# jewettaij/visfd

Hardware: AMD Instinct MI355X
Metric: Mvoxels/s (Gauss+DoG+TV pipeline) on 1024^3 float32; % HBM roofline (higher is better)
Workload: dtype f32

## Files before the change

visfd_amd/build.py:

```python
import concurrent.futures
import os
import subprocess
import sys
import time

HERE = os.path.dirname(os.path.abspath(__file__))
ROOT = os.path.dirname(HERE)
CSRC = os.path.join(HERE, "csrc")
OBJDIR = os.path.join(ROOT, "build", "visfd_hip")
LIB = os.path.join(HERE, "libvisfd_hip.so")

SOURCES = ["host_math.cpp", "blob_post.cpp", "connect.cpp", "watershed_host.cpp", "context.hip", "api.hip", "blob_job.hip", "gauss.hip", "blob.hip", "select.hip", "tv.hip", "resample.hip", "slab.hip", "morph.hip", "extrema.hip", "filter3d.hip", "draw.hip", "watershed.hip", "median.hip", "intensity.hip", "distance.hip"]
TV_VARIANT = [("tv_tiled.hip", "tv_tiled", ["-fno-slp-vectorize"]), ("tv_box.hip", "tv_box", ["-fno-slp-vectorize"]),
              ("tv_list.hip", "tv_list", ["-fno-slp-vectorize"]),
              ("ridge.hip", "ridge", [])]
VARIANTS = TV_VARIANT + [("gauss_fused.hip", "gauss_fused_h%d" % h, ["-DVH_FUSED_H=%d" % h, "-fno-slp-vectorize"])
                         for h in range(1, 9)]
HEADERS = ["common.hpp", "tv_common.hpp", "eigen3.hpp", "union_find.hpp", "tile.hpp", "watershed_host.hpp", "intensity.hpp", os.path.join("..", "..", "include", "visfd_hip.h")]

HIPCC = os.environ.get("HIPCC", "/opt/rocm/bin/hipcc")
FLAGS = ["--offload-arch=gfx950", "-O3", "-std=c++17", "-fPIC", "-ffp-contract=off", "-fno-fast-math",
         "-Wall", "-Wno-unused-function"]


def _mtime(p):
    return os.path.getmtime(p) if os.path.exists(p) else 0.0


def _compile(src, obj, extra=()):
    t0 = time.time()
    cmd = [HIPCC] + FLAGS + list(extra) + ["-x", "hip", "-c", os.path.join(CSRC, src), "-o", obj]
    r = subprocess.run(cmd, capture_output=True, text=True)
    return src, r.returncode, r.stdout + r.stderr, time.time() - t0


def build(force=False, jobs=4, verbose=True):
    os.makedirs(OBJDIR, exist_ok=True)
    newest_header = max(_mtime(os.path.join(CSRC, h)) for h in HEADERS)
    todo, objs = [], []
    units = [(s, os.path.splitext(s)[0], []) for s in SOURCES] + VARIANTS
    flagfile = os.path.join(OBJDIR, "flags.txt")
    flagsig = repr((FLAGS, VARIANTS))
    if not os.path.exists(flagfile) or open(flagfile).read() != flagsig:
        force = True
    for s, stem, extra in units:
        obj = os.path.join(OBJDIR, stem + ".o")
        objs.append(obj)
        if force or _mtime(obj) < max(_mtime(os.path.join(CSRC, s)), newest_header):
            todo.append((s, obj, extra))
    if todo:
        with concurrent.futures.ThreadPoolExecutor(max_workers=jobs) as ex:
            for (src, rc, out, dt), (_, obj, _e) in zip(ex.map(lambda a: _compile(*a), todo), todo):
                if verbose:
                    print("[visfd_amd.build] %-22s %5.1fs %s" % (os.path.basename(obj), dt, "ok" if rc == 0 else "FAILED"))
                if rc != 0:
                    sys.stderr.write(out)
                    raise RuntimeError("hipcc failed on " + src)
                elif out.strip() and verbose:
                    sys.stderr.write(out)
    with open(flagfile, "w") as f:
        f.write(flagsig)
    if todo or not os.path.exists(LIB) or _mtime(LIB) < max(_mtime(o) for o in objs):
        cmd = [HIPCC, "--offload-arch=gfx950", "-shared", "-fPIC", "-o", LIB] + objs
        r = subprocess.run(cmd, capture_output=True, text=True)
        if r.returncode != 0:
            sys.stderr.write(r.stdout + r.stderr)
            raise RuntimeError("link failed")
        if verbose:
            print("[visfd_amd.build] linked", LIB)
    build_cli(verbose)
    return LIB


CLI_SRC = os.path.join(HERE, "cli", "filter_mrc.cpp")
CLI_BIN = os.path.join(HERE, "cli", "filter_mrc")


def build_cli(verbose=True):
    deps = [CLI_SRC, os.path.join(HERE, "cli", "mrc.hpp"), os.path.join(HERE, "cli", "settings.hpp"),
            os.path.join(ROOT, "include", "visfd_hip.hpp"), os.path.join(ROOT, "include", "visfd_hip.h"), LIB]
    if os.path.exists(CLI_BIN) and _mtime(CLI_BIN) >= max(_mtime(d) for d in deps):
        return CLI_BIN
    cmd = ["g++", "-std=c++11", "-O2", "-Wall", "-o", CLI_BIN, CLI_SRC, "-L" + HERE, "-lvisfd_hip",
           "-Wl,-rpath,$ORIGIN/..", "-Wl,-rpath,/opt/rocm/lib"]
    r = subprocess.run(cmd, capture_output=True, text=True)
    if r.returncode != 0:
        sys.stderr.write(r.stdout + r.stderr)
        raise RuntimeError("building filter_mrc failed")
    if verbose:
        print("[visfd_amd.build] built", CLI_BIN)
    return CLI_BIN


if __name__ == "__main__":
    j = 4
    if "-j" in sys.argv:
        j = int(sys.argv[sys.argv.index("-j") + 1])
    build(force="--force" in sys.argv, jobs=j)
```

visfd_amd/csrc/api.hip:

```cpp
#include <algorithm>
#include <cmath>
#include <vector>

#include "common.hpp"

namespace vh {

int gauss_dev(visfd_hip_ctx* ctx, const float* src, float* dst, const float* mask, i64 nx, i64 ny, i64 nz,
              const float sigma[3], const int hw[3], bool normalize, const GaussOpts& o) {
  VH_REQUIRE(ctx && src && dst && sigma && hw, "null argument");
  std::vector<float> t[3];
  for (int d = 0; d < 3; d++) {
    VH_REQUIRE(sigma[d] >= 0.0f, "sigma must be non-negative");
    VH_REQUIRE(hw[d] >= 0 && hw[d] <= MAX_HALFWIDTH, "filter halfwidth must be in [0, 64]");
    t[d].resize(2 * hw[d] + 1);
    host_gauss_taps(sigma[d], hw[d], t[d].data());
  }
  return dev_separable3d(ctx, src, dst, mask, nx, ny, nz, t[0].data(), hw[0], t[1].data(), hw[1], t[2].data(), hw[2],
                         normalize, o);
}

static int dog_dev(visfd_hip_ctx* ctx, const float* src, float* dst, const float* mask, i64 nx, i64 ny, i64 nz,
                   const float sa[3], const float sb[3], const int hw[3], float scale, float* A, float* B) {
  VH_TRY(gauss_dev(ctx, src, dst, mask, nx, ny, nz, sa, hw, true, {A}));
  return gauss_dev(ctx, src, dst, mask, nx, ny, nz, sb, hw, true, {B, dst, scale});
}

LogPlan plan_log(const float sigma[3], float delta, float ratio) {
  LogPlan p;
  for (int d = 0; d < 3; d++) {
    p.sa[d] = (float)(sigma[d] * (1.0 - 0.5 * delta));
    p.sb[d] = (float)(sigma[d] * (1.0 + 0.5 * delta));
    p.hw[d] = (int)std::floor(ratio * std::fmax(p.sa[d], p.sb[d]));
  }
  p.scale = (float)(1.0 / (delta * delta));
  return p;
}

int log_dev(visfd_hip_ctx* ctx, const float* src, float* dst, const float* mask, i64 nx, i64 ny, i64 nz,
            const float sigma[3], float delta, float ratio, float* A, float* B) {
  const LogPlan p = plan_log(sigma, delta, ratio);
  for (int d = 0; d < 3; d++)
    VH_REQUIRE(p.hw[d] >= 0 && p.hw[d] <= MAX_HALFWIDTH, "LoG filter halfwidth must be in [0, 64]");
  float a = 0, b = 0;
  VH_TRY(dog_dev(ctx, src, dst, mask, nx, ny, nz, p.sa, p.sb, p.hw, p.scale, &a, &b));
  if (A) *A = a * p.scale;
  if (B) *B = b * p.scale;
  return VISFD_HIP_OK;
}

namespace {

void halfwidths_from_ratio(const float sigma[3], float ratio, int hw[3]) {
  for (int d = 0; d < 3; d++) {
    hw[d] = (int)std::floor(sigma[d] * ratio);
    if (hw[d] < 1) hw[d] = 1;
  }
}

int gauss_iso_dev(visfd_hip_ctx* ctx, const float* src, float* dst, const float* mask, i64 nx, i64 ny, i64 nz, float sigma,
                  float ratio, bool normalize, const char* what, float** out = nullptr) {
  const int hwv = (int)std::floor(sigma * ratio);
  VH_REQUIRE(hwv >= 0 && hwv <= MAX_HALFWIDTH, std::string(what) + " must be in [0, 64]");
  if (!dst) VH_TRY(ws(ctx, WS_D, (size_t)(nx * ny * nz), &dst));
  if (out) *out = dst;
  const float sg[3] = {sigma, sigma, sigma};
  const int hw[3] = {hwv, hwv, hwv};
  return gauss_dev(ctx, src, dst, mask, nx, ny, nz, sg, hw, normalize);
}

int calc_hessian_dev(visfd_hip_ctx* ctx, const float* src, float* grad, float* hess, const float* mask,
                     i64 nx, i64 ny, i64 nz, float sigma, float ratio) {
  VH_REQUIRE(ctx && src, "null argument");
  VH_TRY(check_dims(nx, ny, nz));
  float* S = nullptr;
  VH_TRY(gauss_iso_dev(ctx, src, nullptr, mask, nx, ny, nz, sigma, ratio, true, "filter halfwidth", &S));
  return dev_hessian(ctx, S, mask, nx, ny, nz, sigma, grad, hess);
}

GaussOpts field_opts(const visfd_hip_ctx* ctx, float* A_out) {
  GaussOpts o;
  o.A_out = A_out;
  o.fma = ctx->opt.gauss_fma != 0;
  return o;
}

bool overlaps(const float* a, const float* b, i64 n) { return a && b && a < b + n && b < a + n; }

int morph_check(visfd_hip_ctx* ctx, const float* src, float* dst, const float* mask, i64 nx, i64 ny, i64 nz, int op,
                int max_op) {
  VH_REQUIRE(ctx && src && dst, "null argument");
  VH_REQUIRE(op >= 0 && op <= max_op, "unknown morphology op");
  VH_TRY(check_dims(nx, ny, nz));
  VH_REQUIRE(!overlaps(src, dst, nx * ny * nz), "morphology cannot run in place (dst overlaps src)");
  VH_REQUIRE(!overlaps(mask, dst, nx * ny * nz), "morphology: dst overlaps mask");
  VH_HIP(hipSetDevice(ctx->device));
  return VISFD_HIP_OK;
}

int median_check(visfd_hip_ctx* ctx, const float* src, float* dst, const float* mask, i64 nx, i64 ny, i64 nz) {
  VH_REQUIRE(ctx && src && dst, "null argument");
  VH_TRY(check_dims(nx, ny, nz));
  VH_REQUIRE(!overlaps(src, dst, nx * ny * nz), "the median filter cannot run in place (dst overlaps src)");
  VH_REQUIRE(!overlaps(mask, dst, nx * ny * nz), "median: dst overlaps mask");
  VH_HIP(hipSetDevice(ctx->device));
  return VISFD_HIP_OK;
// ... 674 lines not shown
```

visfd_amd/csrc/common.hpp:

```cpp
#pragma once

#include <hip/hip_runtime.h>

#include <cstdint>
#include <cstdio>
#include <cstring>
#include <string>
#include <vector>

#include "../../include/visfd_hip.h"

namespace vh {

typedef int64_t i64;

void set_error(const std::string& msg);
int fail(int code, const std::string& msg);

#define VH_HIP(expr)                                                                         \
  do {                                                                                       \
    hipError_t _e = (expr);                                                                  \
    if (_e != hipSuccess)                                                                    \
      return vh::fail(_e == hipErrorOutOfMemory ? VISFD_HIP_ENOMEM : VISFD_HIP_EDEVICE,      \
                      std::string(#expr) + ": " + hipGetErrorString(_e));                    \
  } while (0)

#define VH_TRY(expr)           \
  do {                         \
    int _rc = (expr);          \
    if (_rc != VISFD_HIP_OK) return _rc; \
  } while (0)

#define VH_REQUIRE(cond, msg) \
  do {                        \
    if (!(cond)) return vh::fail(VISFD_HIP_EINVAL, msg); \
  } while (0)

enum Slot {
  WS_A = 0, WS_B, WS_C, WS_D,
  WS_DEN_A, WS_DEN_B,
  WS_NORM,
  WS_LOG0, WS_LOG1, WS_LOG2,
  WS_CAND, WS_COUNTER,
  WS_SCANCNT,
  WS_HIST,
  WS_TVTAB,
  WS_TVAUX,
  WS_TVSCRATCH,
  WS_TVLIST,
  WS_H2D_0, WS_H2D_1, WS_H2D_2, WS_H2D_3, WS_H2D_4,
  WS_MORPH_TAB,
  WS_MORPH_SRC,
  WS_MORPH_TMP,
  WS_EXT_FLAGS,
  WS_EXT_PARENT,
  WS_EXT_COUNT,
  WS_EXT_COUNTERS,
  WS_EXT_LIST,
  WS_EXT_RANKS,
  WS_F3D_TAB,
  WS_DRAW_OWNER,
  WS_DRAW_TAB,
  WS_WSH_KIND,
  WS_WSH_LINK,
  WS_WSH_C,
  WS_WSH_STATE,
  WS_WSH_SEEDS,
  WS_WSH_FLAGS,
  WS_MEDIAN_TAB,
  WS_INTENSITY,
  WS_DIST_DSQ,
  WS_DIST_STACK,
  WS_DIST_POINTS,
  WS_NSLOTS
};

struct BlobJob;

}

struct visfd_hip_options {
  int gauss_3pass = 0;
  int gauss_cfg = 0;
  int gauss_wg_per_cu = 2;
  int tv_dense = 0;
  int tv_fma = 0;
  int gauss_fma = 0;
  int eig_f32 = 0;
  int tv_zrun = 0;
  int tv_no_replay = 0;
  int tv_exact_tiled = 0;
  int tv_no_fold = 0;
  int tv_poison = 0;
  int tv_reserve_wg = 0;
  int tv_max_wg = 0;
  int64_t blob_test_cap = 0;
  int morph_general = 0;
  int filter3d_general = 0;
  int median_general = 0;
  int distance_general = 0;
  int watershed_host = 0;
  int stats_blocks = 0;
  int draw_time = 0;
  int debug = 0;
};

struct visfd_hip_ctx {
  visfd_hip_options opt;
  float* tv_table_dev = nullptr;
  float tv_table_key[2] = {0.0f, 0.0f};
  int tv_table_h = -1;
  int device = 0;
  hipStream_t stream = nullptr;
  bool own_stream = false;
  void* slot_ptr[vh::WS_NSLOTS] = {};
  size_t slot_bytes[vh::WS_NSLOTS] = {};
  int num_cus = 256;
  hipStream_t aux_stream = nullptr;
  std::vector<int> morph_tab;
  int morph_last_path = -1;
  std::vector<float> f3d_raw;
  int64_t f3d_key[5] = {};
  int64_t f3d_n = 0;
  int64_t f3d_ncols = 0;
  float f3d_den = 0.0f;
  int f3d_last_path = -1;
  std::vector<int> median_tab;
  int median_last_path = -1;
  int distance_last_path = -1;
  float draw_ms[3] = {-1.0f, -1.0f, -1.0f};
  int64_t wsh_stats[4] = {-1, -1, -1, -1};
  std::vector<vh::BlobJob*> blob_jobs;
};

namespace vh {

int blob_jobs_drain(visfd_hip_ctx* ctx, const BlobJob* except = nullptr);
void blob_jobs_abort(visfd_hip_ctx* ctx);

int ws_get(visfd_hip_ctx* ctx, Slot s, size_t bytes, void** out);
template <typename T>
inline int ws(visfd_hip_ctx* ctx, Slot s, size_t count, T** out) {
  void* p = nullptr;
  int rc = ws_get(ctx, s, count * sizeof(T), &p);
  *out = static_cast<T*>(p);
  return rc;
}

inline int check_dims(i64 nx, i64 ny, i64 nz) {
  if (nx <= 0 || ny <= 0 || nz <= 0) return fail(VISFD_HIP_EINVAL, "image dimensions must be positive");
  return VISFD_HIP_OK;
}
inline bool overlap_bytes(const void* a, size_t na, const void* b, size_t nb) {
  const char* p = static_cast<const char*>(a);
  const char* q = static_cast<const char*>(b);
  return p && q && p < q + nb && q < p + na;
}
inline int check_dims32(i64 nx, i64 ny, i64 nz) {
  if (nx >= (1LL << 31) || ny >= (1LL << 31) || nz >= (1LL << 31)) return fail(VISFD_HIP_EINVAL, "dimension too large");
  return VISFD_HIP_OK;
}

constexpr int MAX_HALFWIDTH = 64;
struct Taps {
  float t[2 * MAX_HALFWIDTH + 1];
  int h;
};

void host_gauss_taps(float sigma, int h, float* t);
void host_conv_ones(i64 n, const float* t, int h, float* out);
int host_tv_halfwidth(float sigma, float cutoff);
void host_tv_tables(float sigma, int h, float* w, float* rhat);
float host_gengauss3d_peak(const float width[3], float m_exp, float ratio);
void host_gengauss3d_table(const float width[3], float m_exp, const int hw[3], float* table_out, float* A_out);
void host_gengauss3d_halfwidths(const float width[3], float m_exp, float ratio, float threshold, int hw[3]);
i64 host_dogg3d_table(const float width_a[3], const float width_b[3], float m_exp, float n_exp, float ratio,
                      float threshold, int hw[3], float* table_out, i64 cap, float* A_out, float* B_out);
i64 host_sphere_structure(float radius, float radius_max, float bmax, int* dxyz, float* b, i64 cap);

struct GaussOpts {
  float* A_out = nullptr;
  const float* minuend = nullptr;
  float log_scale = 1.0f;
  bool fma = false;
  i64 z_lo = 0, nz_global = 0;
};
int dev_separable3d(visfd_hip_ctx* ctx, const float* src, float* dst, const float* mask, i64 nx, i64 ny, i64 nz,
                    const float* tx, int hx, const float* ty, int hy, const float* tz, int hz, bool normalize,
                    const GaussOpts& o = {});

struct GaussRequest {
  const float* src;
  float* dst;
  i64 nx, ny, nz;
  Taps tx, ty, tz;
  const float *Dx, *Dy, *Dz;
  i64 dz_offset;
  bool normalize;
  bool zpass;
  const float* minuend;
  float log_scale;
  bool fma;
  const float* numer;
};

int gauss_dev(visfd_hip_ctx* ctx, const float* src, float* dst, const float* mask, i64 nx, i64 ny, i64 nz,
              const float sigma[3], const int hw[3], bool normalize, const GaussOpts& o = {});
struct LogPlan {
  float sa[3], sb[3], scale;
  int hw[3];
};
LogPlan plan_log(const float sigma[3], float delta, float ratio);
int log_dev(visfd_hip_ctx* ctx, const float* src, float* dst, const float* mask, i64 nx, i64 ny, i64 nz,
            const float sigma[3], float delta, float ratio, float* A, float* B);
int dev_sub_square(visfd_hip_ctx* ctx, const float* a, const float* b, float* out, i64 n);
int dev_scale_clamp_sqrt(visfd_hip_ctx* ctx, float* a_inout, i64 n, float scale);

struct ScanPending {
  const unsigned long long* counters = nullptr;
  const void* survivors = nullptr;
  size_t cap_idx = 0, cap_out = 0;
};
int blob_scan_launch(visfd_hip_ctx* ctx, const BlobJob* owner, int set, hipEvent_t done, const float* lo, const float* mid,
                     const float* hi, const float* mask, i64 nx, i64 ny, i64 nz, float min_thr, float max_thr,
                     ScanPending* pending);
int blob_scan_collect(visfd_hip_ctx* ctx, const ScanPending& pending, hipEvent_t done, hipStream_t aux, i64 nx, i64 ny,
                      int scale_index,
                      float sigma, std::vector<visfd_hip_blob>* minima, std::vector<visfd_hip_blob>* maxima,
                      bool* overflow);
int dev_blob_scan(visfd_hip_ctx* ctx, const float* lo, const float* mid, const float* hi,
                  const float* mask, i64 nx, i64 ny, i64 nz, int scale_index, float sigma,
                  float min_thr, float max_thr, bool want_min, bool want_max,
                  std::vector<visfd_hip_blob>* minima, std::vector<visfd_hip_blob>* maxima);

int dev_hessian(visfd_hip_ctx* ctx, const float* smoothed, const float* mask, i64 nx, i64 ny, i64 nz,
                float sigma, float* grad_planar, float* hess_planar);
int dev_hessian_saliency(visfd_hip_ctx* ctx, const float* hess_planar, const float* mask, i64 nvox,
                         int order, float* saliency, float* dir_planar);
int dev_ridge_saliency_fused(visfd_hip_ctx* ctx, const float* smoothed, const float* mask, i64 nx,
                             i64 ny, i64 nz, float sigma, int order, float* saliency,
                             float* dir_planar);
int dev_ridge_score(visfd_hip_ctx* ctx, const float* smoothed, const float* mask, i64 nx, i64 ny, i64 nz,
                    float sigma, int order, float* saliency, const float* peak_img = nullptr, const float* peak_bg = nullptr);
int dev_ridge_directions(visfd_hip_ctx* ctx, const float* smoothed, const float* saliency, i64 nx, i64 ny, i64 nz,
                         float sigma, int order, float* dir_planar);
int dev_diagonalize(visfd_hip_ctx* ctx, const float* m6_planar, float* out6_planar, i64 n, int order);
int dev_tensor_saliency(visfd_hip_ctx* ctx, const float* tensor_planar, const float* mask, i64 nvox,
                        int order, float* saliency, const float* peak_img = nullptr, const float* peak_bg = nullptr);

int dev_select_histogram(visfd_hip_ctx* ctx, const float* sal, const float* mask, i64 nvox, int pass,
                         uint32_t prefix, uint64_t* hist_host, uint64_t* n_unmasked_host);
int dev_select_histogram_todev(visfd_hip_ctx* ctx, const float* sal, const float* mask, i64 nvox, int pass, uint32_t prefix,
                               uint64_t* hist_dev);
int dev_apply_threshold(visfd_hip_ctx* ctx, float* sal, i64 nvox, float thr);
int dev_threshold_fraction(visfd_hip_ctx* ctx, float* sal, const float* mask, i64 nvox, float fraction,
                           float* thr_out);

int dev_tv_dense_stick(visfd_hip_ctx* ctx, const float* sal, const float* dir_planar,
                       float* tensor_planar, const float* mask_src, const float* mask_dst, i64 nx,
                       i64 ny, i64 nz, i64 z_out0, i64 z_out1, float sigma_tv, int exponent,
                       float cutoff, bool curves);

int dev_tv_weight_sum(visfd_hip_ctx* ctx, const float* sal, float* den, const float* mask_src, const float* mask_dst, i64 nx,
                      i64 ny, i64 nz, float sigma_tv, float cutoff);

constexpr int MORPH_RUN_MAX_R = 10;
struct MorphElem {
  i64 n = 0;
  int lo[3] = {0, 0, 0}, hi[3] = {0, 0, 0};
  bool flat = true;
  bool runs = false;
  int R = 0;
  signed char run_len[(2 * MORPH_RUN_MAX_R + 1) * (2 * MORPH_RUN_MAX_R + 1)];
};

int dev_morph_table(visfd_hip_ctx* ctx, const float* src, float* dst, const float* mask, i64 nx, i64 ny, i64 nz,
                    const MorphElem& el, bool dilate, int epi, bool nan_masked, int* path);
int dev_nan_masked(visfd_hip_ctx* ctx, const float* src, const float* mask, float* out, i64 n);
int morph_put_table(visfd_hip_ctx* ctx, const int* dxyz, const float* b, i64 n, MorphElem* el);
int morph_run(visfd_hip_ctx* ctx, const float* src, float* dst, const float* mask, i64 nx, i64 ny, i64 nz, int op,
              MorphElem el);

struct MedianTab {
  i64 n = 0;
  int lo[3] = {0, 0, 0}, hi[3] = {0, 0, 0};
  int W = 0, H = 0, D = 0;
};
int median_put_table(visfd_hip_ctx* ctx, const int* dxyz, i64 n, MedianTab* mt);
// ... 93 lines not shown
```

visfd_amd/csrc/context.hip:

```cpp
#include <cctype>
#include <cstdlib>

#include "common.hpp"

namespace vh {

static thread_local std::string g_last_error;
void set_error(const std::string& msg) { g_last_error = msg; }
int fail(int code, const std::string& msg) {
  g_last_error = msg;
  return code;
}

int ws_get(visfd_hip_ctx* ctx, Slot s, size_t bytes, void** out) {
  if (bytes == 0) bytes = 16;
  if (ctx->slot_bytes[s] < bytes) {
    if (ctx->slot_ptr[s] && (s == WS_CAND || s == WS_SCANCNT)) VH_TRY(blob_jobs_drain(ctx));
    if (ctx->slot_ptr[s]) {
      VH_HIP(hipStreamSynchronize(ctx->stream));
      VH_HIP(hipFree(ctx->slot_ptr[s]));
      ctx->slot_ptr[s] = nullptr;
      ctx->slot_bytes[s] = 0;
    }
    void* p = nullptr;
    hipError_t e = hipMalloc(&p, bytes);
    if (e != hipSuccess)
      return fail(VISFD_HIP_ENOMEM, "hipMalloc of " + std::to_string(bytes) + " bytes failed: " +
                                        hipGetErrorString(e));
    ctx->slot_ptr[s] = p;
    ctx->slot_bytes[s] = bytes;
  }
  *out = ctx->slot_ptr[s];
  return VISFD_HIP_OK;
}

namespace {

struct OptionDesc { const char* name; int visfd_hip_options::*i; int64_t visfd_hip_options::*l; };
const OptionDesc kOptions[] = {
    {"gauss_3pass", &visfd_hip_options::gauss_3pass, nullptr},   {"gauss_cfg", &visfd_hip_options::gauss_cfg, nullptr},
    {"gauss_wg_per_cu", &visfd_hip_options::gauss_wg_per_cu, nullptr}, {"tv_dense", &visfd_hip_options::tv_dense, nullptr},
    {"tv_zrun", &visfd_hip_options::tv_zrun, nullptr}, {"tv_fma", &visfd_hip_options::tv_fma, nullptr},
    {"gauss_fma", &visfd_hip_options::gauss_fma, nullptr}, {"eig_f32", &visfd_hip_options::eig_f32, nullptr},
    {"tv_no_replay", &visfd_hip_options::tv_no_replay, nullptr}, {"tv_max_wg", &visfd_hip_options::tv_max_wg, nullptr},
    {"tv_poison", &visfd_hip_options::tv_poison, nullptr}, {"tv_no_fold", &visfd_hip_options::tv_no_fold, nullptr}, {"tv_exact_tiled", &visfd_hip_options::tv_exact_tiled, nullptr}, {"tv_reserve_wg", &visfd_hip_options::tv_reserve_wg, nullptr},
    {"blob_test_cap", nullptr, &visfd_hip_options::blob_test_cap}, {"debug", &visfd_hip_options::debug, nullptr},
    {"morph_general", &visfd_hip_options::morph_general, nullptr},
    {"filter3d_general", &visfd_hip_options::filter3d_general, nullptr},
    {"median_general", &visfd_hip_options::median_general, nullptr},
    {"distance_general", &visfd_hip_options::distance_general, nullptr},
    {"draw_time", &visfd_hip_options::draw_time, nullptr},
    {"stats_blocks", &visfd_hip_options::stats_blocks, nullptr},
    {"watershed_host", &visfd_hip_options::watershed_host, nullptr},
};
bool set_option(visfd_hip_options* o, const char* name, int64_t value) {
  for (const OptionDesc& d : kOptions) {
    if (std::strcmp(d.name, name) != 0) continue;
    if (d.i) o->*(d.i) = (int)value; else o->*(d.l) = value;
    return true;
  }
  return false;
}
bool get_option(const visfd_hip_options* o, const char* name, int64_t* value) {
  for (const OptionDesc& d : kOptions) {
    if (std::strcmp(d.name, name) != 0) continue;
    *value = d.i ? (int64_t)(o->*(d.i)) : o->*(d.l);
    return true;
  }
  return false;
}
void options_from_environment(visfd_hip_options* o) {
  for (const OptionDesc& d : kOptions) {
    std::string env = "VISFD_HIP_";
    for (const char* c = d.name; *c; c++) env += (char)std::toupper((unsigned char)*c);
    if (const char* e = std::getenv(env.c_str())) set_option(o, d.name, (int64_t)std::atoll(e));
  }
}

void forget_slot_caches(visfd_hip_ctx* ctx) {
  ctx->tv_table_dev = nullptr;
  ctx->tv_table_h = -1;
  ctx->morph_tab.clear();
  ctx->f3d_raw.clear();
  ctx->median_tab.clear();
}

}
}

using namespace vh;

extern "C" {

int visfd_hip_abi_version(void) { return 10; }
const char* visfd_hip_last_error(void) { return g_last_error.c_str(); }

int visfd_hip_create(int device, void* stream, visfd_hip_ctx** out) {
  VH_REQUIRE(out, "null output pointer");
  int count = 0;
  hipError_t e = hipGetDeviceCount(&count);
  if (e != hipSuccess || count <= 0)
    return fail(VISFD_HIP_EDEVICE, "no HIP device available (libvisfd_hip has no CPU fallback)");
  VH_REQUIRE(device >= 0 && device < count, "bad device ordinal");
  VH_HIP(hipSetDevice(device));
  hipDeviceProp_t prop;
  VH_HIP(hipGetDeviceProperties(&prop, device));
  visfd_hip_ctx* ctx = new visfd_hip_ctx();
  ctx->device = device;
  ctx->num_cus = prop.multiProcessorCount > 0 ? prop.multiProcessorCount : 256;
  options_from_environment(&ctx->opt);
  if (stream) {
    ctx->stream = (hipStream_t)stream;
    ctx->own_stream = false;
  } else {
    e = hipStreamCreateWithFlags(&ctx->stream, hipStreamNonBlocking);
    if (e != hipSuccess) {
      delete ctx;
      return fail(VISFD_HIP_EDEVICE, std::string("hipStreamCreate: ") + hipGetErrorString(e));
    }
    ctx->own_stream = true;
  }
  *out = ctx;
  return VISFD_HIP_OK;
}

int visfd_hip_set_option(visfd_hip_ctx* ctx, const char* name, int64_t value) {
  VH_REQUIRE(ctx && name, "null argument");
  if (!set_option(&ctx->opt, name, value)) return fail(VISFD_HIP_EINVAL, std::string("unknown option: ") + name);
  return VISFD_HIP_OK;
}

int visfd_hip_get_option(visfd_hip_ctx* ctx, const char* name, int64_t* value) {
  VH_REQUIRE(ctx && name && value, "null argument");
  if (!get_option(&ctx->opt, name, value)) return fail(VISFD_HIP_EINVAL, std::string("unknown option: ") + name);
  return VISFD_HIP_OK;
}
// ... 57 lines not shown
```

visfd_amd/csrc/gauss.hip:

```cpp
#include <cstdlib>

#include "common.hpp"

#define VH_STREAM_STORE(v, p) __builtin_nontemporal_store((v), (p))

namespace vh {

namespace {

constexpr int BLOCK = 256;

enum { NORM_NONE = 0, NORM_BOX = 1, NORM_DEN = 2 };

constexpr int MARCH_T = 128;
constexpr int MARCH_X = 64;

template <int HT>
struct TapsK {
  float t[2 * (HT > 0 ? HT : 1) + 1];
};

template <int HT, bool MASKED>
__global__ void __launch_bounds__(BLOCK)
conv_march_kernel(const float* __restrict__ in, float* __restrict__ out, const float* __restrict__ mask,
// ... 215 lines not shown
    return fail(VISFD_HIP_EINVAL, "filter halfwidth must be in [0, 64]");
  std::memset(T, 0, sizeof(Taps));
  T->h = h;
  for (int k = 0; k < 2 * h + 1; k++) T->t[k] = t[k];
  return VISFD_HIP_OK;
}

template <int HT>
TapsK<HT> taps_k(const Taps& T) {
  TapsK<HT> k;
  for (int i = 0; i < 2 * (HT > 0 ? HT : 1) + 1; i++) k.t[i] = HT > 0 ? T.t[i] : 0.0f;
  return k;
}

#define VH_FOR_H(h, ...)                                                                            \
  switch (h) {                                                                                      \
    case 1: { constexpr int HT = 1; __VA_ARGS__; } break;   case 2: { constexpr int HT = 2; __VA_ARGS__; } break;   \
    case 3: { constexpr int HT = 3; __VA_ARGS__; } break;   case 4: { constexpr int HT = 4; __VA_ARGS__; } break;   \
    case 5: { constexpr int HT = 5; __VA_ARGS__; } break;   case 6: { constexpr int HT = 6; __VA_ARGS__; } break;   \
    case 7: { constexpr int HT = 7; __VA_ARGS__; } break;   case 8: { constexpr int HT = 8; __VA_ARGS__; } break;   \
    case 9: { constexpr int HT = 9; __VA_ARGS__; } break;   case 10: { constexpr int HT = 10; __VA_ARGS__; } break; \
    default: { constexpr int HT = 0; __VA_ARGS__; } break;                                                 \
  }

template <bool MASKED>
int launch_march(visfd_hip_ctx* ctx, int axis, const float* in, float* out, const float* mask, float* den_out,
                 const Taps& T, i64 nx, i64 ny, i64 nz) {
  const i64 plane = nx * ny;
  const int n_march = (int)(axis == 1 ? ny : nz), n_other = (int)(axis == 1 ? nz : ny);
  const i64 stride_march = axis == 1 ? nx : plane, stride_other = axis == 1 ? plane : nx;
  const int xblocks = (int)((nx + MARCH_X - 1) / MARCH_X), mblocks = (n_march + MARCH_T - 1) / MARCH_T;
  const i64 nblk = (i64)xblocks * mblocks * n_other;
  if (nblk > 0x7fffffffLL) return fail(VISFD_HIP_EINVAL, "volume too large for one launch");
  const size_t lds = sizeof(float) * (size_t)(MARCH_T + 2 * T.h) * MARCH_X * (MASKED ? 2 : 1);
  VH_FOR_H(T.h, {
    auto kern = conv_march_kernel<HT, MASKED>;
    if (lds > 48 * 1024)
      VH_HIP(hipFuncSetAttribute(reinterpret_cast<const void*>(kern), hipFuncAttributeMaxDynamicSharedMemorySize, (int)lds));
    kern<<<dim3((unsigned)nblk), dim3(BLOCK), lds, ctx->stream>>>(in, out, mask, den_out, taps_k<HT>(T), T, (int)nx, n_march,
                                                                  n_other, stride_march, stride_other, xblocks, mblocks);
  })
  VH_HIP(hipGetLastError());
  return VISFD_HIP_OK;
}

template <int NORM>
int launch_row(visfd_hip_ctx* ctx, const float* in, float* out, const float* den_in, const float* Dx, const float* Dy,
               const float* Dz, i64 dz_offset, const Taps& T, i64 nx, i64 ny, i64 nz, const float* minuend = nullptr,
               float log_scale = 1.0f) {
  const int xblocks = (int)((nx + ROW_X - 1) / ROW_X), yblocks = (int)((ny + ROW_Y - 1) / ROW_Y);
  const i64 nblk = (i64)xblocks * yblocks * nz;
  if (nblk > 0x7fffffffLL) return fail(VISFD_HIP_EINVAL, "volume too large for one launch");
  const size_t lds = sizeof(float) * (size_t)ROW_Y * (ROW_X + 2 * T.h);
  VH_FOR_H(T.h, {
    conv_row_kernel<HT, NORM><<<dim3((unsigned)nblk), dim3(BLOCK), lds, ctx->stream>>>(
        in, out, den_in, Dx, Dy, Dz, dz_offset, taps_k<HT>(T), T, (int)nx, (int)ny, (int)nz, xblocks, yblocks, minuend,
        log_scale);
  })
  VH_HIP(hipGetLastError());
  return VISFD_HIP_OK;
}

}

typedef int FusedLaunch(visfd_hip_ctx* ctx, const GaussRequest& rq);
FusedLaunch launch_gauss_fused_h1, launch_gauss_fused_h2, launch_gauss_fused_h3, launch_gauss_fused_h4, launch_gauss_fused_h5,
    launch_gauss_fused_h6, launch_gauss_fused_h7, launch_gauss_fused_h8;
static FusedLaunch* const fused_launch[9] = {nullptr, launch_gauss_fused_h1, launch_gauss_fused_h2, launch_gauss_fused_h3,
                                             launch_gauss_fused_h4, launch_gauss_fused_h5, launch_gauss_fused_h6,
                                             launch_gauss_fused_h7, launch_gauss_fused_h8};

static bool fused_applies(const visfd_hip_ctx* ctx, const GaussRequest& rq) {
  const int H = rq.tx.h;
  if (ctx->opt.gauss_3pass || H < 1 || H > 8 || rq.ty.h != H || (rq.zpass && rq.tz.h != H)) return false;
  if (rq.nx * rq.ny >= (1LL << 29) || rq.nz >= (1LL << 31)) return false;
  if (rq.src == rq.dst || rq.numer == rq.dst) return false;
  const Taps* const axis[3] = {&rq.tx, &rq.ty, &rq.tz};
  for (int a = 0; a < (rq.zpass ? 3 : 2); a++)
    for (int j = 1; j <= H; j++)
      if (std::memcmp(&axis[a]->t[H + j], &axis[a]->t[H - j], sizeof(float)) != 0) return false;
  return true;
}

constexpr int GAUSS_DECLINED = -1;
static int gauss_fused_route(visfd_hip_ctx* ctx, const GaussRequest& rq) {
  return fused_applies(ctx, rq) ? fused_launch[rq.tx.h](ctx, rq) : GAUSS_DECLINED;
}

int dev_separable3d(visfd_hip_ctx* ctx, const float* src, float* dst, const float* mask, i64 nx, i64 ny, i64 nz,
                    const float* tx, int hx, const float* ty, int hy, const float* tz, int hz, bool normalize,
                    const GaussOpts& o) {
  VH_TRY(check_dims(nx, ny, nz));
  GaussRequest rq = {};
  rq.src = src; rq.dst = dst; rq.nx = nx; rq.ny = ny; rq.nz = nz;
  VH_TRY(fill_taps(&rq.tx, tx, hx));
  VH_TRY(fill_taps(&rq.ty, ty, hy));
  VH_TRY(fill_taps(&rq.tz, tz, hz));
  if (o.A_out) *o.A_out = (tx[hx] * ty[hy]) * tz[hz];
  rq.dz_offset = o.z_lo;
  rq.normalize = normalize; rq.zpass = true;
  rq.minuend = o.minuend; rq.log_scale = o.log_scale;
  rq.fma = o.fma && !o.minuend;
  const Taps &Tx = rq.tx, &Ty = rq.ty, &Tz = rq.tz;
  const float* const minuend = o.minuend;
  const float log_scale = o.log_scale;
  const i64 n = nx * ny * nz;

  if (normalize && !mask) {
    float* D = nullptr;
    const i64 nz_global = o.nz_global ? o.nz_global : nz;
    const i64 total = nx + ny + nz_global;
    VH_TRY(ws(ctx, WS_NORM, (size_t)total, &D));
    norm_lines_kernel<<<dim3((unsigned)((total + BLOCK - 1) / BLOCK)), dim3(BLOCK), 0, ctx->stream>>>(D, nx, ny, nz_global, Tx, Ty, Tz);
    VH_HIP(hipGetLastError());
    rq.Dx = D; rq.Dy = D + nx; rq.Dz = D + nx + ny;
  }

  if (!mask) {
    const int rc = gauss_fused_route(ctx, rq);
    if (rc != GAUSS_DECLINED) return rc;
  }

  float *A = nullptr, *B = nullptr;
  VH_TRY(ws(ctx, WS_A, (size_t)n, &A));
  VH_TRY(ws(ctx, WS_B, (size_t)n, &B));
  if (nx >= (1LL << 31) || ny >= (1LL << 31) || nz >= (1LL << 31)) return fail(VISFD_HIP_EINVAL, "image dimension too large");
  if (!mask) {
    VH_TRY(launch_march<false>(ctx, 2, src, A, nullptr, nullptr, Tz, nx, ny, nz));
    VH_TRY(launch_march<false>(ctx, 1, A, B, nullptr, nullptr, Ty, nx, ny, nz));
    if (normalize) return launch_row<NORM_BOX>(ctx, B, dst, nullptr, rq.Dx, rq.Dy, rq.Dz, rq.dz_offset, Tx, nx, ny, nz, minuend, log_scale);
    return launch_row<NORM_NONE>(ctx, B, dst, nullptr, nullptr, nullptr, nullptr, 0, Tx, nx, ny, nz, minuend, log_scale);
  }
  GaussRequest yx = rq;
  yx.src = A; yx.zpass = false; yx.normalize = false; yx.fma = false;
  if (!normalize) {
    VH_TRY(launch_march<true>(ctx, 2, src, A, mask, nullptr, Tz, nx, ny, nz));
    const int rc = gauss_fused_route(ctx, yx);
    if (rc != GAUSS_DECLINED) return rc;
    VH_TRY(launch_march<false>(ctx, 1, A, B, nullptr, nullptr, Ty, nx, ny, nz));
    return launch_row<NORM_NONE>(ctx, B, dst, nullptr, nullptr, nullptr, nullptr, 0, Tx, nx, ny, nz, minuend, log_scale);
  }
  float *DA = nullptr, *DB = nullptr;
  VH_TRY(ws(ctx, WS_DEN_A, (size_t)n, &DA));
  VH_TRY(ws(ctx, WS_DEN_B, (size_t)n, &DB));
  VH_TRY(launch_march<true>(ctx, 2, src, A, mask, DA, Tz, nx, ny, nz));
  yx.src = DA; yx.numer = B;
  if (fused_applies(ctx, yx)) {
    GaussRequest num = yx;
    num.src = A; num.dst = B; num.numer = nullptr; num.minuend = nullptr; num.log_scale = 1.0f;
    VH_TRY(fused_launch[Tx.h](ctx, num));
    return fused_launch[Tx.h](ctx, yx);
  }
  VH_TRY(launch_march<false>(ctx, 1, A, B, nullptr, nullptr, Ty, nx, ny, nz));
  VH_TRY(launch_march<false>(ctx, 1, DA, DB, nullptr, nullptr, Ty, nx, ny, nz));
  VH_TRY(launch_row<NORM_NONE>(ctx, DB, DA, nullptr, nullptr, nullptr, nullptr, 0, Tx, nx, ny, nz));
  return launch_row<NORM_DEN>(ctx, B, dst, DA, nullptr, nullptr, nullptr, 0, Tx, nx, ny, nz, minuend, log_scale);
}

int dev_sub_square(visfd_hip_ctx* ctx, const float* a, const float* b, float* out, i64 n) {
  const unsigned g = grid_for(n, BLOCK, (i64)ctx->num_cus * 16);
  sub_square_kernel<<<dim3(g), dim3(BLOCK), 0, ctx->stream>>>(a, b, out, n);
  VH_HIP(hipGetLastError());
  return VISFD_HIP_OK;
}

int dev_scale_clamp_sqrt(visfd_hip_ctx* ctx, float* a, i64 n, float scale) {
  const unsigned g = grid_for(n, BLOCK, (i64)ctx->num_cus * 16);
  scale_clamp_sqrt_kernel<<<dim3(g), dim3(BLOCK), 0, ctx->stream>>>(a, n, scale);
  VH_HIP(hipGetLastError());
  return VISFD_HIP_OK;
}

}
```

Before: 2460.

## Fuse both DoG Gaussian blurs into a shared-input pair z and yx pass

Adds a paired DoG path for halfwidths 7 to 10 (6 is compiled but off by default). A z-pass kernel reads the source once and writes both z-blurred volumes. A combined y+x kernel then blurs both, normalizes, subtracts and scales, and writes the DoG output directly. This replaces two independent 3D Gaussians plus a subtraction pass, cutting source reads and intermediate traffic. The cost is a second full-size temporary volume, heavier register and LDS use per block, and a table that gates which halfwidths take the new path.

New measurement: 2555 (median of 6 runs). 1.04x the previous value.

```diff
diff --git a/visfd_amd/build.py b/visfd_amd/build.py
--- a/visfd_amd/build.py
+++ b/visfd_amd/build.py
@@ -14,7 +14,8 @@
 TV_VARIANT = [("tv_tiled.hip", "tv_tiled", ["-fno-slp-vectorize"]), ("tv_box.hip", "tv_box", ["-fno-slp-vectorize"]),
               ("tv_list.hip", "tv_list", ["-fno-slp-vectorize"]),
               ("ridge.hip", "ridge", [])]
-VARIANTS = TV_VARIANT + [("gauss_fused.hip", "gauss_fused_h%d" % h, ["-DVH_FUSED_H=%d" % h, "-fno-slp-vectorize"])
+PAIR_FLAGS = ["-fno-slp-vectorize"]
+VARIANTS = TV_VARIANT + [("gauss_pair.hip", "gauss_pair", PAIR_FLAGS)] + [("gauss_fused.hip", "gauss_fused_h%d" % h, ["-DVH_FUSED_H=%d" % h, "-fno-slp-vectorize"])
                          for h in range(1, 9)]
 HEADERS = ["common.hpp", "tv_common.hpp", "eigen3.hpp", "union_find.hpp", "tile.hpp", "watershed_host.hpp", "intensity.hpp", os.path.join("..", "..", "include", "visfd_hip.h")]
 
diff --git a/visfd_amd/csrc/api.hip b/visfd_amd/csrc/api.hip
--- a/visfd_amd/csrc/api.hip
+++ b/visfd_amd/csrc/api.hip
@@ -20,8 +20,30 @@
                          normalize, o);
 }
 
+static int log_pair_try(visfd_hip_ctx* ctx, const float* src, float* dst, i64 nx, i64 ny, i64 nz, const float sa[3],
+                        const float sb[3], const int hw[3], float scale, float* A, float* B) {
+  if (!ctx || !src || !dst || !sa || !sb || !hw || ctx->opt.log_pair == 0) return GAUSS_DECLINED;
+  LogPairRequest rq = {};
+  rq.src = src; rq.dst = dst; rq.nx = nx; rq.ny = ny; rq.nz = nz; rq.scale = scale;
+  for (int d = 0; d < 3; d++) {
+    if (!(sa[d] >= 0.0f) || !(sb[d] >= 0.0f) || hw[d] < 0 || hw[d] > MAX_HALFWIDTH) return GAUSS_DECLINED;
+    rq.a[d].h = rq.b[d].h = hw[d];
+    host_gauss_taps(sa[d], hw[d], rq.a[d].t);
+    host_gauss_taps(sb[d], hw[d], rq.b[d].t);
+  }
+  const int rc = log_pair_route(ctx, rq);
+  if (rc != VISFD_HIP_OK) return rc;
+  if (A) *A = (rq.a[0].t[hw[0]] * rq.a[1].t[hw[1]]) * rq.a[2].t[hw[2]];
+  if (B) *B = (rq.b[0].t[hw[0]] * rq.b[1].t[hw[1]]) * rq.b[2].t[hw[2]];
+  return VISFD_HIP_OK;
+}
+
 static int dog_dev(visfd_hip_ctx* ctx, const float* src, float* dst, const float* mask, i64 nx, i64 ny, i64 nz,
                    const float sa[3], const float sb[3], const int hw[3], float scale, float* A, float* B) {
+  if (!mask) {
+    const int rc = log_pair_try(ctx, src, dst, nx, ny, nz, sa, sb, hw, scale, A, B);
+    if (rc != GAUSS_DECLINED) return rc;
+  }
   VH_TRY(gauss_dev(ctx, src, dst, mask, nx, ny, nz, sa, hw, true, {A}));
   return gauss_dev(ctx, src, dst, mask, nx, ny, nz, sb, hw, true, {B, dst, scale});
 }
diff --git a/visfd_amd/csrc/common.hpp b/visfd_amd/csrc/common.hpp
--- a/visfd_amd/csrc/common.hpp
+++ b/visfd_amd/csrc/common.hpp
@@ -83,6 +83,8 @@
   int gauss_3pass = 0;
   int gauss_cfg = 0;
   int gauss_wg_per_cu = 2;
+  int log_pair = 1;
+  int log_pair_chunk = 0;
   int tv_dense = 0;
   int tv_fma = 0;
   int gauss_fma = 0;
@@ -204,6 +206,19 @@
   const float* numer;
 };
 
+constexpr int GAUSS_DECLINED = -1;
+int dev_norm_lines(visfd_hip_ctx* ctx, float* D, i64 nx, i64 ny, i64 nz, const Taps& tx, const Taps& ty, const Taps& tz);
+
+struct LogPairRequest {
+  const float* src;
+  float* dst;
+  i64 nx, ny, nz;
+  Taps a[3], b[3];
+  float scale;
+  i64 z_lo, nz_global;
+};
+int log_pair_route(visfd_hip_ctx* ctx, const LogPairRequest& rq);
+
 int gauss_dev(visfd_hip_ctx* ctx, const float* src, float* dst, const float* mask, i64 nx, i64 ny, i64 nz,
               const float sigma[3], const int hw[3], bool normalize, const GaussOpts& o = {});
 struct LogPlan {
diff --git a/visfd_amd/csrc/context.hip b/visfd_amd/csrc/context.hip
--- a/visfd_amd/csrc/context.hip
+++ b/visfd_amd/csrc/context.hip
@@ -52,6 +52,8 @@
     {"draw_time", &visfd_hip_options::draw_time, nullptr},
     {"stats_blocks", &visfd_hip_options::stats_blocks, nullptr},
     {"watershed_host", &visfd_hip_options::watershed_host, nullptr},
+    {"log_pair", &visfd_hip_options::log_pair, nullptr},
+    {"log_pair_chunk", &visfd_hip_options::log_pair_chunk, nullptr},
 };
 bool set_option(visfd_hip_options* o, const char* name, int64_t value) {
   for (const OptionDesc& d : kOptions) {
diff --git a/visfd_amd/csrc/gauss.hip b/visfd_amd/csrc/gauss.hip
--- a/visfd_amd/csrc/gauss.hip
+++ b/visfd_amd/csrc/gauss.hip
@@ -321,9 +321,15 @@
   return true;
 }
 
-constexpr int GAUSS_DECLINED = -1;
 static int gauss_fused_route(visfd_hip_ctx* ctx, const GaussRequest& rq) {
   return fused_applies(ctx, rq) ? fused_launch[rq.tx.h](ctx, rq) : GAUSS_DECLINED;
+}
+
+int dev_norm_lines(visfd_hip_ctx* ctx, float* D, i64 nx, i64 ny, i64 nz, const Taps& tx, const Taps& ty, const Taps& tz) {
+  const i64 total = nx + ny + nz;
+  norm_lines_kernel<<<dim3((unsigned)((total + BLOCK - 1) / BLOCK)), dim3(BLOCK), 0, ctx->stream>>>(D, nx, ny, nz, tx, ty, tz);
+  VH_HIP(hipGetLastError());
+  return VISFD_HIP_OK;
 }
 
 int dev_separable3d(visfd_hip_ctx* ctx, const float* src, float* dst, const float* mask, i64 nx, i64 ny, i64 nz,
@@ -350,8 +356,7 @@
     const i64 nz_global = o.nz_global ? o.nz_global : nz;
     const i64 total = nx + ny + nz_global;
     VH_TRY(ws(ctx, WS_NORM, (size_t)total, &D));
-    norm_lines_kernel<<<dim3((unsigned)((total + BLOCK - 1) / BLOCK)), dim3(BLOCK), 0, ctx->stream>>>(D, nx, ny, nz_global, Tx, Ty, Tz);
-    VH_HIP(hipGetLastError());
+    VH_TRY(dev_norm_lines(ctx, D, nx, ny, nz_global, Tx, Ty, Tz));
     rq.Dx = D; rq.Dy = D + nx; rq.Dz = D + nx + ny;
   }
 
diff --git a/visfd_amd/csrc/gauss_pair.hip b/visfd_amd/csrc/gauss_pair.hip
--- /dev/null
+++ b/visfd_amd/csrc/gauss_pair.hip
@@ -0,0 +1,321 @@
+#include <type_traits>
+
+#include "common.hpp"
+
+namespace vh {
+
+namespace {
+
+constexpr int Z_NT = 256;
+constexpr int Z_PF = 8;
+constexpr int YX_NT = 256;
+constexpr int YX_PF = 12;
+constexpr int Z_CHUNK = 256;
+constexpr int Y_CHUNK = 512;
+
+template <int H>
+struct PairTaps {
+  float a[H + 1], b[H + 1];
+};
+
+template <int B, int E, class F>
+__device__ __forceinline__ void static_for(F&& f) {
+  if constexpr (B < E) {
+    f(std::integral_constant<int, B>{});
+    static_for<B + 1, E>(f);
+  }
+}
+
+template <int H>
+__device__ __forceinline__ void taps_to_vgprs(const PairTaps<H>& tp, float (&ta)[H + 1], float (&tb)[H + 1]) {
+#pragma unroll
+  for (int m = 0; m <= H; m++) {
+    ta[m] = tp.a[m];
+    tb[m] = tp.b[m];
+    asm volatile("" : "+v"(ta[m]));
+    asm volatile("" : "+v"(tb[m]));
+  }
+}
+
+template <int H, int U>
+__device__ __forceinline__ void scatter(float (&ring)[2 * H + 1], const float (&t)[H + 1], float x) {
+  constexpr int W = 2 * H + 1;
+  float pr[H + 1];
+#pragma unroll
+  for (int m = 0; m <= H; m++) pr[m] = t[m] * x;
+#pragma unroll
+  for (int j = -H; j <= H; j++) {
+    const int s = (U + H - j) % W;
+    if (j == -H) ring[s] = pr[H];
+    else ring[s] = ring[s] + pr[j < 0 ? -j : j];
+    asm volatile("" : "+v"(ring[s]));
+  }
+}
+
+template <int H>
+__global__ void __launch_bounds__(Z_NT, 4)
+pair_z_kernel(const float* __restrict__ src, float* __restrict__ za, float* __restrict__ zb, PairTaps<H> tp, i64 plane, int nz,
+              int zchunk) {
+  constexpr int W = 2 * H + 1;
+  const i64 c = (i64)blockIdx.x * Z_NT + threadIdx.x;
+  if (c >= plane) return;
+  float ta[H + 1], tb[H + 1];
+  taps_to_vgprs<H>(tp, ta, tb);
+  const int zs = blockIdx.y * zchunk;
+  const int ze = min(zs + zchunk, nz);
+  const int nsteps = ze - zs + 2 * H;
+  const int ktop = ze - 1 + H;
+  const float* p = src + c;
+  auto load = [&](int s) -> float { return p[(i64)min(max(ktop - s, 0), nz - 1) * plane]; };
+  auto inside = [&](int s) -> bool { return ktop - s >= 0 && ktop - s < nz; };
+  float ra[W], rb[W], q[Z_PF];
+#pragma unroll
+  for (int m = 0; m < W; m++) ra[m] = rb[m] = 0.0f;
+#pragma unroll
+  for (int i = 0; i < Z_PF; i++) q[i] = load(i);
+#pragma nounroll
+  for (int nb = 0; nb < nsteps; nb += W) {
+    static_for<0, W>([&](auto U) {
+      constexpr int u = decltype(U)::value;
+      const int s = nb + u;
+      const float x = inside(s) ? q[0] : 0.0f;
+#pragma unroll
+      for (int i = 0; i + 1 < Z_PF; i++) q[i] = q[i + 1];
+      q[Z_PF - 1] = load(s + Z_PF);
+      scatter<H, u>(ra, ta, x);
+      scatter<H, u>(rb, tb, x);
+      const int z = ktop + H - s;
+      const bool done = s >= 2 * H && z >= zs;
+      const i64 o = done ? (i64)z * plane : 0;
+      const int len = done ? (int)(plane * 4) : 0;
+      const __amdgpu_buffer_rsrc_t sa = __builtin_amdgcn_make_buffer_rsrc((void*)(za + o), 0, len, 0x00020000);
+      const __amdgpu_buffer_rsrc_t sb = __builtin_amdgcn_make_buffer_rsrc((void*)(zb + o), 0, len, 0x00020000);
+      __builtin_amdgcn_raw_buffer_store_b32(__builtin_bit_cast(unsigned, ra[u]), sa, (int)c * 4, 0, 2);
+      __builtin_amdgcn_raw_buffer_store_b32(__builtin_bit_cast(unsigned, rb[u]), sb, (int)c * 4, 0, 2);
+      __builtin_amdgcn_sched_barrier(0);
+    });
+  }
+}
+
+template <int H>
+struct YxCfg {
+  static constexpr int W = 2 * H + 1;
+  static constexpr int XW = (2 * H + 4 + 3) / 4;
+  static constexpr int TX = YX_NT + 4 - 4 * XW;
+  static constexpr int QPR = TX / 4;
+  static_assert(TX % 4 == 0 && TX + 2 * H <= YX_NT && TX > 0, "tile width");
+  static_assert(sizeof(float) * 2 * W * YX_NT <= 64 * 1024, "LDS rows of both filters");
+};
+
+template <int H>
+__global__ void __launch_bounds__(YX_NT, 3)
+pair_yx_kernel(const float* __restrict__ za, const float* __restrict__ zb, float* __restrict__ dst, PairTaps<H> tp,
+               const float* __restrict__ Da, const float* __restrict__ Db, i64 dz_offset, int nx, int ny, int ychunk,
+               int xtiles, int ychunks, float scale, int vec_ok) {
+  typedef YxCfg<H> C;
+  constexpr int W = C::W;
+  __shared__ __attribute__((aligned(16))) float sA[W][YX_NT];
+  __shared__ __attribute__((aligned(16))) float sB[W][YX_NT];
+  float ta[H + 1], tb[H + 1];
+  taps_to_vgprs<H>(tp, ta, tb);
+  unsigned b = blockIdx.x;
+  const int bx = b % xtiles;
+  b /= xtiles;
+  const int by = b % ychunks;
+  const int z = b / ychunks;
+  const int tid = threadIdx.x;
+  const int x0 = bx * C::TX;
+  const int xc = x0 - H + tid;
+  const bool col_ok = xc >= 0 && xc < nx;
+  const int ys = by * ychunk;
+  const int ye = min(ys + ychunk, ny);
+  const int nsteps = ye - ys + 2 * H;
+  const int ktop = ye - 1 + H;
+  const i64 zoff = (i64)z * nx * ny;
+  const float* pa = za + zoff + min(max(xc, 0), nx - 1);
+  const float* pb = zb + zoff + min(max(xc, 0), nx - 1);
+  auto row_off = [&](int s) -> i64 { return (i64)min(max(ktop - s, 0), ny - 1) * nx; };
+  auto inside = [&](int s) -> bool { return col_ok && ktop - s >= 0 && ktop - s < ny; };
+  float ra[W], rb[W], qa[YX_PF], qb[YX_PF];
+#pragma unroll
+  for (int m = 0; m < W; m++) ra[m] = rb[m] = 0.0f;
+#pragma unroll
+  for (int i = 0; i < YX_PF; i++) {
+    qa[i] = pa[row_off(i)];
+    qb[i] = pb[row_off(i)];
+  }
+  const float* Dax = Da; const float* Day = Da + nx; const float* Daz = Da + nx + ny + dz_offset;
+  const float* Dbx = Db; const float* Dby = Db + nx; const float* Dbz = Db + nx + ny + dz_offset;
+  const float daz = Daz[z], dbz = Dbz[z];
+  float* const out_plane = dst + zoff;
+
+#pragma nounroll
+  for (int nb = 0; nb < nsteps; nb += W) {
+    static_for<0, W>([&](auto U) {
+      constexpr int u = decltype(U)::value;
+      const int s = nb + u;
+      const bool in = inside(s);
+      const float xa = in ? qa[0] : 0.0f, xb = in ? qb[0] : 0.0f;
+#pragma unroll
+      for (int i = 0; i + 1 < YX_PF; i++) { qa[i] = qa[i + 1]; qb[i] = qb[i + 1]; }
+      qa[YX_PF - 1] = pa[row_off(s + YX_PF)];
+      qb[YX_PF - 1] = pb[row_off(s + YX_PF)];
+      scatter<H, u>(ra, ta, xa);
+      scatter<H, u>(rb, tb, xb);
+      sA[u][tid] = ra[u];
+      sB[u][tid] = rb[u];
+      __builtin_amdgcn_sched_barrier(0);
+    });
+    __syncthreads();
+    for (int task = tid; task < W * C::QPR; task += YX_NT) {
+      const int u = task / C::QPR, qd = task - u * C::QPR;
+      const int s = nb + u;
+      const int y = ktop + H - s;
+      const int x = x0 + 4 * qd;
+      if (s < 2 * H || y < ys || x >= nx) continue;
+      float ga[4], gb[4];
+      {
+        float v[4 * C::XW];
+#pragma unroll
+        for (int k = 0; k < C::XW; k++) {
+          const float4 t4 = *reinterpret_cast<const float4*>(&sA[u][4 * qd + 4 * k]);
+          v[4 * k] = t4.x; v[4 * k + 1] = t4.y; v[4 * k + 2] = t4.z; v[4 * k + 3] = t4.w;
+        }
+#pragma unroll
+        for (int jj = 0; jj < W; jj++) {
+          const float t = ta[jj < H ? H - jj : jj - H];
+#pragma unroll
+          for (int k = 0; k < 4; k++) {
+            const float term = t * v[2 * H - jj + k];
+            ga[k] = jj == 0 ? term : ga[k] + term;
+          }
+        }
+      }
+      {
+        float v[4 * C::XW];
+#pragma unroll
+        for (int k = 0; k < C::XW; k++) {
+          const float4 t4 = *reinterpret_cast<const float4*>(&sB[u][4 * qd + 4 * k]);
+          v[4 * k] = t4.x; v[4 * k + 1] = t4.y; v[4 * k + 2] = t4.z; v[4 * k + 3] = t4.w;
+        }
+#pragma unroll
+        for (int jj = 0; jj < W; jj++) {
+          const float t = tb[jj < H ? H - jj : jj - H];
+#pragma unroll
+          for (int k = 0; k < 4; k++) {
+            const float term = t * v[2 * H - jj + k];
+            gb[k] = jj == 0 ? term : gb[k] + term;
+          }
+        }
+      }
+      float da[4], db[4];
+      const float day = Day[y], dby = Dby[y];
+      bool ones = true;
+#pragma unroll
+      for (int k = 0; k < 4; k++) {
+        const int xi = min(x + k, nx - 1);
+        ga[k] = ga[k] + 0.0f;
+        gb[k] = gb[k] + 0.0f;
+        da[k] = (Dax[xi] * day) * daz;
+        db[k] = (Dbx[xi] * dby) * dbz;
+        ones = ones && da[k] == 1.0f && db[k] == 1.0f;
+      }
+      if (__builtin_amdgcn_ballot_w64(!ones) != 0ull) {
+#pragma unroll
+        for (int k = 0; k < 4; k++) {
+          ga[k] = ga[k] / da[k];
+          gb[k] = gb[k] / db[k];
+        }
+      }
+      float r[4];
+#pragma unroll
+      for (int k = 0; k < 4; k++) {
+        const float dd = ga[k] - gb[k];
+        r[k] = dd * scale;
+      }
+      float* o = out_plane + (i64)y * nx + x;
+      if (vec_ok && x + 3 < nx) {
+        typedef float v4f __attribute__((ext_vector_type(4)));
+        const v4f r4 = {r[0], r[1], r[2], r[3]};
+        __builtin_nontemporal_store(r4, reinterpret_cast<v4f*>(o));
+      } else {
+#pragma unroll
+        for (int k = 0; k < 4; k++)
+          if (x + k < nx) __builtin_nontemporal_store(r[k], &o[k]);
+      }
+    }
+    __syncthreads();
+  }
+}
+
+constexpr int PAIR_H_MIN = 6, PAIR_H_MAX = 10;
+const bool kPairWins[PAIR_H_MAX + 1] = {false, false, false, false, false, false,  false,  true,  true,
+                                         true,  true};
+
+bool bit_symmetric(const Taps& T) {
+  for (int j = 1; j <= T.h; j++)
+    if (std::memcmp(&T.t[T.h + j], &T.t[T.h - j], sizeof(float)) != 0) return false;
+  return true;
+}
+bool same_bits(const Taps& A, const Taps& B) {
+  return A.h == B.h && std::memcmp(A.t, B.t, sizeof(float) * (2 * A.h + 1)) == 0;
+}
+
+template <int H>
+int launch_pair(visfd_hip_ctx* ctx, const LogPairRequest& rq, const float* Da, const float* Db) {
+  typedef YxCfg<H> C;
+  const i64 nx = rq.nx, ny = rq.ny, nz = rq.nz, plane = nx * ny, n = plane * nz;
+  float *za = nullptr, *zb = nullptr;
+  VH_TRY(ws(ctx, WS_A, (size_t)n, &za));
+  VH_TRY(ws(ctx, WS_B, (size_t)n, &zb));
+  PairTaps<H> tz, tyx;
+  for (int m = 0; m <= H; m++) {
+    tz.a[m] = rq.a[2].t[H + m];  tz.b[m] = rq.b[2].t[H + m];
+    tyx.a[m] = rq.a[0].t[H + m]; tyx.b[m] = rq.b[0].t[H + m];
+  }
+  const int opt_chunk = ctx->opt.log_pair_chunk;
+  i64 zchunk = opt_chunk > 0 ? opt_chunk : Z_CHUNK;
+  if ((nz + zchunk - 1) / zchunk > 65535) zchunk = (nz + 65534) / 65535;
+  const i64 zblocks = (plane + Z_NT - 1) / Z_NT, zchunks = (nz + zchunk - 1) / zchunk;
+  const i64 ychunk = opt_chunk > 0 ? opt_chunk : Y_CHUNK;
+  const i64 xtiles = (nx + C::TX - 1) / C::TX, ychunks = (ny + ychunk - 1) / ychunk;
+  const i64 yxblocks = xtiles * ychunks * nz;
+  if (zblocks > 0x7fffffffLL || yxblocks > 0x7fffffffLL) return fail(VISFD_HIP_EINVAL, "volume too large for one launch");
+  pair_z_kernel<H><<<dim3((unsigned)zblocks, (unsigned)zchunks), dim3(Z_NT), 0, ctx->stream>>>(rq.src, za, zb, tz, plane, (int)nz,
+                                                                                                (int)zchunk);
+  VH_HIP(hipGetLastError());
+  const int vec_ok = ((nx & 3) == 0) && ((reinterpret_cast<uintptr_t>(rq.dst) & 15) == 0);
+  pair_yx_kernel<H><<<dim3((unsigned)yxblocks), dim3(YX_NT), 0, ctx->stream>>>(za, zb, rq.dst, tyx, Da, Db, rq.z_lo, (int)nx, (int)ny,
+                                                                                (int)ychunk, (int)xtiles, (int)ychunks, rq.scale,
+                                                                                vec_ok);
+  VH_HIP(hipGetLastError());
+  return VISFD_HIP_OK;
+}
+
+}
+
+int log_pair_route(visfd_hip_ctx* ctx, const LogPairRequest& rq) {
+  const int mode = ctx->opt.log_pair;
+  const int H = rq.a[0].h;
+  if (mode == 0 || ctx->opt.gauss_3pass || H < PAIR_H_MIN || H > PAIR_H_MAX) return GAUSS_DECLINED;
+  if (mode == 1 && !kPairWins[H]) return GAUSS_DECLINED;
+  if (rq.nx <= 0 || rq.ny <= 0 || rq.nz <= 0 || rq.nx * rq.ny >= (1LL << 29) || rq.nz >= (1LL << 31)) return GAUSS_DECLINED;
+  for (int d = 0; d < 3; d++)
+    if (rq.a[d].h != H || rq.b[d].h != H || !bit_symmetric(rq.a[d]) || !bit_symmetric(rq.b[d])) return GAUSS_DECLINED;
+  if (!same_bits(rq.a[0], rq.a[1]) || !same_bits(rq.b[0], rq.b[1])) return GAUSS_DECLINED;
+  const i64 nz_global = rq.nz_global ? rq.nz_global : rq.nz;
+  const i64 lines = rq.nx + rq.ny + nz_global;
+  float* D = nullptr;
+  VH_TRY(ws(ctx, WS_NORM, (size_t)(2 * lines), &D));
+  VH_TRY(dev_norm_lines(ctx, D, rq.nx, rq.ny, nz_global, rq.a[0], rq.a[1], rq.a[2]));
+  VH_TRY(dev_norm_lines(ctx, D + lines, rq.nx, rq.ny, nz_global, rq.b[0], rq.b[1], rq.b[2]));
+  switch (H) {
+    case 6: return launch_pair<6>(ctx, rq, D, D + lines);
+    case 7: return launch_pair<7>(ctx, rq, D, D + lines);
+    case 8: return launch_pair<8>(ctx, rq, D, D + lines);
+    case 9: return launch_pair<9>(ctx, rq, D, D + lines);
+    default: return launch_pair<10>(ctx, rq, D, D + lines);
+  }
+}
+
+}
```
